# MaxMax2016/MixGAN-TTS

Hardware: AMD Instinct MI355X
Metric: denoiser steps/sec (80-mel, L=1000 frames, B=16 per GPU) (higher is better)
Workload: dtype f32

## Files before the change

mixgan-tts_amd/csrc/denoiser.hip:

```cpp
#include "denoiser_common.h"
#include "resblock_fused.h"
#include "resblock_split.h"
#include "pointwise_fused.h"
#include "denoiser_persist.h"
#include "denoiser_persist16.h"
#include "denoiser_team16.h"
#include <atomic>
#include <cstdlib>
#include <cstring>

struct EpiCond {
    struct Params {
        float *out;
        const float *bias;
        const float *x;
        const float *vec;
        int C;
    };
    template <int WM, int NNB>
    static __device__ __forceinline__ void run(const Params &p, f32x16 (&acc)[WM][NNB], int b, int mrow0, int l0w,
                                               int lane, int Lout)
    {
        const int h = lane >> 5, c = lane & 31;
#pragma unroll
// ... 401 lines not shown
    a.sig_save = sig_save;
    a.tnh_save = tnh_save;
    a.L = L;
    a.first = 1;
    const bool vec4 = (L % 4 == 0) && (((uintptr_t)cond & 15) == 0);
    launch_res_layer(a, B, L, nsave == 4, vec4, (hipStream_t)stream);
    MG_LAUNCH_CHECK();
    return MG_OK;
}

struct PostSample {
    const float *coef1, *coef2, *logvar;
    const float *noise;
    unsigned long long seed, noise_stream;
    float *x0_out;
    int n_steps, clip;
    const float *cproj;
    float *cproj_out;
    const float *step_vectors;
    int step_index, step_count;
};

static unsigned *g_host_err = nullptr, *g_host_err_dev = nullptr;
static std::atomic<int> g_host_err_state{0};

unsigned *mg_host_err_device_ptr()
{
    int s = g_host_err_state.load();
    if (s == 0) {
        static std::atomic_flag busy = ATOMIC_FLAG_INIT;
        if (busy.test_and_set()) return nullptr;
        void *h = nullptr, *dptr = nullptr;
        if (hipHostMalloc(&h, 64, hipHostMallocMapped | hipHostMallocPortable) == hipSuccess && h) {
            std::memset(h, 0, 64);
            if (hipHostGetDevicePointer(&dptr, h, 0) == hipSuccess && dptr) {
                g_host_err = (unsigned *)h;
                g_host_err_dev = (unsigned *)dptr;
                g_host_err_state.store(1);
            } else {
                (void)hipHostFree(h);
            }
        }
        (void)hipGetLastError();
        busy.clear();
        s = g_host_err_state.load();
    }
    return s == 1 ? g_host_err_dev : nullptr;
}

extern "C" unsigned mg_persist_error(int clear)
{
    if (g_host_err_state.load() != 1) {
        (void)mg_host_err_device_ptr();
        if (g_host_err_state.load() != 1) return 0u;
    }
    const unsigned v = __atomic_load_n(g_host_err, __ATOMIC_ACQUIRE);
    if (clear && v) __atomic_store_n(g_host_err, 0u, __ATOMIC_RELEASE);
    return v;
}

int mg_device_cus()
{
    static std::atomic<int> cus[64];
    int dev = 0;
    if (hipGetDevice(&dev) != hipSuccess || dev < 0 || dev >= 64) return 256;
    int n = cus[dev].load();
    if (n == 0) {
        if (hipDeviceGetAttribute(&n, hipDeviceAttributeMultiprocessorCount, dev) != hipSuccess || n <= 0) n = 256;
        cus[dev].store(n);
    }
    return n;
}

unsigned mg_persist_spin_limit()
{
    if (const char *e = std::getenv("MG_PERSIST_SPIN_LIMIT")) {
        const long v = std::atol(e);
        if (v > 0) return (unsigned)v;
    }
    return DP_SPIN_LIMIT;
}
static unsigned long long *g_persist_dbg = nullptr;
extern "C" void mg_debug_persist_stamps(unsigned long long *device_buffer) { g_persist_dbg = device_buffer; }

struct StepVecAt {
    size_t emb, h1pre, h1, s, dvec, hvec, total;
};
static inline StepVecAt den_stepvec_layout(const mg_denoiser_dims *d, size_t rows)
{
    const size_t C = d->channels, NL = d->n_layers;
    StepVecAt w;
    size_t p = 0;
    auto take = [&](size_t n) {
        size_t at = p;
        p += mg_align_up(n, 64);
        return at;
    };
    w.emb = take(rows * C);
    w.h1pre = take(rows * 4 * C);
    w.h1 = take(rows * 4 * C);
    w.s = take(rows * C);
    w.dvec = take(NL * rows * C);
    w.hvec = d->multi_speaker ? take(NL * rows * C) : w.dvec;
    w.total = p;
    return w;
}

template <class At>
static int den_step_vectors(const mg_denoiser_dims *d, const DenLayout &o, const float *packed, const int64_t *t,
                            const float *spk, float *ws, const At &w, int B, hipStream_t st, int spk_rows = 0)
{
    const int C = d->channels, H = d->cond_channels, NL = d->n_layers;
    const float *lay0 = packed + o.layers;
    hipLaunchKernelGGL(step_embed_kernel, dim3(mg_cdiv(B * (C / 2), 256)), dim3(256), 0, st, t, packed + o.freq,
                       ws + w.emb, B, C);
    MG_LAUNCH_CHECK();
    MG_TRY(small_linear(packed + o.mlp0, 0, ws + w.emb, ws + w.h1, 0, nullptr, 0, ws + w.h1pre, B, 4 * C, C, 1, 1, st));
    MG_TRY(small_linear(packed + o.mlp2, 0, ws + w.h1, ws + w.s, 0, nullptr, 0, nullptr, B, C, 4 * C, 1, 0, st));
    MG_TRY(small_linear(lay0 + o.l_wd, (long)o.layer_stride, ws + w.s, ws + w.dvec, (long)B * C, nullptr, 0, nullptr, B,
                        C, C, NL, 0, st));
    if (d->multi_speaker)
        MG_TRY(small_linear(lay0 + o.l_wp, (long)o.layer_stride, spk, ws + w.hvec, (long)B * C, ws + w.dvec,
                            (long)B * C, nullptr, B, C, H, NL, 0, st, spk_rows));
    return MG_OK;
}

extern "C" size_t mg_denoiser_step_vectors_floats(const mg_denoiser_dims *d, int n, int B)
{
    if (den_check(d) != MG_OK || n <= 0 || B <= 0) return 0;
    return den_stepvec_layout(d, (size_t)n * B).total;
}

extern "C" int mg_denoiser_step_vectors(const mg_denoiser_dims *d, const float *packed, const int64_t *t, const float *spk,
                                        float *vectors, size_t vectors_floats, int n, int B, void *stream)
{
    MG_TRY(den_check(d));
    if (!packed || !t || !vectors) return MG_ERR_ARG;
    if (d->multi_speaker && !spk) return MG_ERR_ARG;
    if (n <= 0 || B <= 0) return MG_ERR_SHAPE;
    const StepVecAt w = den_stepvec_layout(d, (size_t)n * B);
    if (vectors_floats < w.total) return MG_ERR_WORKSPACE;
    const DenLayout o = den_layout(d, 0);
    return den_step_vectors(d, o, packed, t, spk, vectors, w, n * B, (hipStream_t)stream, B);
}

static int denoiser_forward(const mg_denoiser_dims *d, const float *packed, const float *x_t, const int64_t *t,
                            const float *cond, const float *spk, float *out, float *ws, size_t ws_floats, int B,
                            int L, int mode, const PostSample *post, void *stream);

extern "C" int mg_denoiser_fwd(const mg_denoiser_dims *d, const float *packed, const float *x_t, const int64_t *t,
                               const float *cond, const float *spk, float *out, float *ws, size_t ws_floats, int B,
                               int L, int mode, void *stream)
{
    return denoiser_forward(d, packed, x_t, t, cond, spk, out, ws, ws_floats, B, L, mode, nullptr, stream);
}

extern "C" int mg_denoiser_psample(const mg_denoiser_dims *d, const float *packed, const float *x_t, const int64_t *t,
                                   const float *cond, const float *spk, const float *coef1, const float *coef2,
                                   const float *logvar, int n_steps, const float *noise, unsigned long long seed,
                                   unsigned long long noise_stream, int clip, float *x_prev, float *x0_out,
                                   const mg_sampling_loop *loop, float *ws, size_t ws_floats, int B, int L, int mode,
                                   void *stream)
{
    const float *cproj = loop ? loop->cproj : nullptr;
    float *cproj_out = loop ? loop->cproj_out : nullptr;
    const float *step_vectors = loop ? loop->step_vectors : nullptr;
// ... 83 lines not shown
struct DenFwdPins {
    int nt;
    int solo;
    int team;
};
static DenFwdPins den_fwd_pins()
{
    const char *ne = std::getenv("MG_PERSIST_NT"), *se = std::getenv("MG_PERSIST_SOLO");
    const char *te = std::getenv("MG_PERSIST_TEAM");
    return DenFwdPins{ne ? std::atoi(ne) : 0, !(se && se[0] == '0'), te ? std::atoi(te) : -1};
}

static DenFwdPlan den_fwd_plan(const mg_denoiser_dims *d, int B, int L, int mode, int cproj_mode, bool loop_vectors,
                               int cus)
{
    const bool save = mode & MG_FWD_SAVE, split = mode & MG_FWD_SPLIT, has_p16 = mode & MG_FWD_P16;
    const int C = d->channels, H = d->cond_channels, M = d->mel_bins, NL = d->n_layers;
    const DenFwdPins pin = den_fwd_pins();
    static const bool force_generic = std::getenv("MG_DENOISER_GENERIC") != nullptr;
    DenFwdPlan p{};
    p.fused = !force_generic && C == RB_C && H == RB_C;
    int nt = (long)mg_cdiv(L, 64) * B > 128 ? 64 : 32;
    if (nt == 32 && has_p16 && !save && (long)mg_cdiv(L, 32) * B <= 128) nt = 16;
    bool wide32 = nt == 32 && save && (long)mg_cdiv(L, 32) * B <= 256;
    bool eight64 = false;
    if (pin.nt == 32 || pin.nt == 64 || pin.nt == 328 || (pin.nt == 16 && has_p16 && !save)) {
        nt = pin.nt == 328 ? 32 : pin.nt;
        wide32 = pin.nt == 328;
    }
    if (pin.nt == 864) {
        nt = 64;
        eight64 = true;
    }
    if (nt == 16 && mg_cdiv(L, 16) > 128) nt = 32;
    if (nt != 32) wide32 = false;
    const bool solo32 = pin.solo && nt == 32 && !wide32 && !save && (long)mg_cdiv(L, 32) * B <= cus &&
                        mg_cdiv(L, 32) <= cus / 4;
    int team = 0;
    if (nt == 16 && !save && den_ws(d, B, L, save).team != 0 && pin.team != 0) {
        const long tiles16 = (long)mg_cdiv(L, 16) * B;
        if (tiles16 * 4 <= cus && pin.team != 2) team = 4;
        else if (tiles16 * 2 <= cus && pin.team != 4) team = 2;
    }
    const bool solo16 = pin.solo && nt == 16 && team == 0 && (long)mg_cdiv(L, 16) * B <= cus && mg_cdiv(L, 16) <= cus / 4;
    p.tiles_per_b = mg_cdiv(L, nt);
    const int chain_cap = (nt == 64 || wide32 || solo32 || solo16) ? cus / 4 : cus / 2;
    const bool persist = p.fused && !split && M <= 96 && den_persist_allowed(NL, p.tiles_per_b, chain_cap);
    p.own_vectors = !(persist && loop_vectors);
    if (!persist) return p;
    mg_fwd_plan &k = p.k;
    k.path = MG_PLAN_SINGLE;
    k.nt = nt;
    k.team = team;
    if (team) {
        k.family = MG_PLAN_TEAM16;
        k.waves = 16 / team;
        k.solo = team == 4;
    } else if (nt == 16) {
        k.family = MG_PLAN_PERSIST16;
        k.waves = 4;
        k.solo = solo16;
    } else {
        k.family = MG_PLAN_PERSIST;
        k.waves = eight64 || wide32 ? 8 : 4;
        k.solo = (nt == 64 && !eight64) || solo32;
    }
    k.cproj_mode = save ? 0 : cproj_mode;
    k.grid = p.tiles_per_b * B * (team ? team : 1);
    k.block = k.waves * 64;
    return p;
}

extern "C" int mg_denoiser_fwd_plan(const mg_denoiser_dims *d, int B, int L, int mode, int cproj_mode, int cus,
                                    mg_fwd_plan *out)
{
    MG_TRY(den_check(d));
    if (!out || cproj_mode < 0 || cproj_mode > 2 || ((mode & MG_FWD_SPLIT) && (mode & MG_FWD_SAVE))) return MG_ERR_ARG;
    if (B <= 0 || L <= 0) return MG_ERR_SHAPE;
    *out = den_fwd_plan(d, B, L, mode, cproj_mode, false, cus > 0 ? cus : mg_device_cus()).k;
    return MG_OK;
}

typedef void (*DenFwdKernel)(PersistArgs);
template <int NT, bool V, bool T, bool S, int NWV, int CPM = 0, bool SOLO = false>
constexpr DenFwdKernel dpk = denoiser_persist_kernel<NT, V, T, S, NWV, CPM, SOLO>;
struct DpForm {
    DenFwdKernel save[2];
    DenFwdKernel cpm[3][2];
    DenFwdKernel timing[3];
};
static const DpForm dp_forms[5] = {
    {{dpk<64, false, false, true, 4>, dpk<64, true, false, true, 4>},
     {{dpk<64, false, false, false, 4, 0>, dpk<64, true, false, false, 4, 0>},
      {dpk<64, false, false, false, 4, 1>, dpk<64, true, false, false, 4, 1>},
      {dpk<64, false, false, false, 4, 2>, dpk<64, true, false, false, 4, 2>}},
     {dpk<64, true, true, false, 4, 0>, nullptr, dpk<64, true, true, false, 4, 2>}},
    {{dpk<64, false, false, true, 8>, dpk<64, true, false, true, 8>},
     {{dpk<64, false, false, false, 8, 0>, dpk<64, true, false, false, 8, 0>},
      {dpk<64, false, false, false, 8, 1>, dpk<64, true, false, false, 8, 1>},
      {dpk<64, false, false, false, 8, 2>, dpk<64, true, false, false, 8, 2>}},
     {dpk<64, true, true, false, 8, 0>, nullptr, nullptr}},
    {{dpk<32, false, false, true, 8>, dpk<32, true, false, true, 8>},
     {{dpk<32, false, false, false, 8, 0>, dpk<32, true, false, false, 8, 0>},
      {dpk<32, false, false, false, 8, 1>, dpk<32, true, false, false, 8, 1>},
      {dpk<32, false, false, false, 8, 2>, dpk<32, true, false, false, 8, 2>}},
     {nullptr, nullptr, nullptr}},
    {{nullptr, nullptr},
     {{dpk<32, false, false, false, 4, 0, true>, dpk<32, true, false, false, 4, 0, true>},
      {dpk<32, false, false, false, 4, 1, true>, dpk<32, true, false, false, 4, 1, true>},
      {dpk<32, false, false, false, 4, 2, true>, dpk<32, true, false, false, 4, 2, true>}},
     {nullptr, nullptr, nullptr}},
    {{dpk<32, false, false, true, 4>, dpk<32, true, false, true, 4>},
     {{dpk<32, false, false, false, 4, 0>, dpk<32, true, false, false, 4, 0>},
      {dpk<32, false, false, false, 4, 1>, dpk<32, true, false, false, 4, 1>},
      {dpk<32, false, false, false, 4, 2>, dpk<32, true, false, false, 4, 2>}},
     {dpk<32, true, true, false, 4, 0>, nullptr, nullptr}},
};
static const DenFwdKernel dp16_kernels[2][2] = {
    {denoiser_persist16_kernel<false, false>, denoiser_persist16_kernel<true, false>},
    {denoiser_persist16_kernel<false, true>, denoiser_persist16_kernel<true, true>}};
static const DenFwdKernel team16_kernels[2][2] = {
    {denoiser_team16_kernel<false, 2>, denoiser_team16_kernel<true, 2>},
    {denoiser_team16_kernel<false, 4>, denoiser_team16_kernel<true, 4>}};

static DenFwdKernel den_fwd_kernel(const mg_fwd_plan &k, bool save, bool stamps, bool vec4)
{
    if (k.family == MG_PLAN_TEAM16) return team16_kernels[k.team == 4][vec4];
    if (k.family == MG_PLAN_PERSIST16) return dp16_kernels[k.solo != 0][vec4];
    const DpForm &f = dp_forms[k.nt == 64 ? (k.waves == 8) : k.waves == 8 ? 2 : k.solo ? 3 : 4];
    if (save) return f.save[vec4];
    if (stamps && vec4 && f.timing[k.cproj_mode]) return f.timing[k.cproj_mode];
    return f.cpm[k.cproj_mode][vec4];
}

struct DpPair {
    int b_split;
    const float *x_t, *cond;
    float *out, *ws;
    const DenWs *w;
};

static PersistArgs den_persist_args(const mg_denoiser_dims *d, const float *packed, const DenLayout &o,
                                    const DenFwdPlan &p, const float *x_t, const int64_t *t, const float *cond,
                                    float *out, float *ws, const DenWs &w, int B, int L, bool save,
                                    const PostSample *post, const DpPair *pair)
{
    const int C = d->channels, NL = d->n_layers;
    const bool p16 = p.k.nt == 16;
    float *const sws = pair ? pair->ws : save ? ws : nullptr;
    const DenWs &sw = pair ? *pair->w : w;
    PersistArgs a;
    a.x_t = x_t;
    a.cond = cond;
    a.cproj = post ? post->cproj : nullptr;
    a.cproj_out = post ? post->cproj_out : nullptr;
    a.in_w = packed + (p16 ? o.in_w16 : o.in_w);
    a.in_b = packed + o.in_b;
    a.layers = packed + o.layers;
    a.layer_stride = o.layer_stride;
    a.l_wc = o.l_wc;
    a.l_w3 = o.l_w3;
    a.l_wo = o.l_wo;
    a.l_bc = o.l_bc;
    a.l_b3 = o.l_b3;
    a.l_bo = o.l_bo;
    a.p16layers = pair ? nullptr : packed + o.p16layers;
    a.p16layer_stride = pair ? 0 : o.p16layer_stride;
    a.p_wc = pair ? 0 : o.p_wc;
    a.p_w3 = pair ? 0 : o.p_w3;
    a.p_wo = pair ? 0 : o.p_wo;
    a.skip_w = packed + (p16 ? o.skip_w16 : o.skip_w);
    a.skip_b = packed + o.skip_b;
    a.out_w = packed + (p16 ? o.out_w16 : o.out_w);
    a.out_b = packed + o.out_b;
    a.hvec = ws + w.hvec;
    a.dvec = ws + w.dvec;
    a.vec_rows = 0;
    if (!p.own_vectors) {
        const StepVecAt v = den_stepvec_layout(d, (size_t)post->step_count * B);
        a.hvec = post->step_vectors + v.hvec + (size_t)post->step_index * B * C;
        a.dvec = post->step_vectors + v.dvec + (size_t)post->step_index * B * C;
        a.vec_rows = post->step_count * B;
    }
    a.out = out;
    a.t = t;
    a.coef1 = post ? post->coef1 : nullptr;
    a.coef2 = post ? post->coef2 : nullptr;
    a.logvar = post ? post->logvar : nullptr;
    a.noise = post ? post->noise : nullptr;
    a.seed = post ? post->seed : 0ull;
    a.noise_stream = post ? post->noise_stream : 0ull;
    a.x0_out = post ? post->x0_out : nullptr;
    a.gran = reinterpret_cast<dp_u64 *>(ws + w.gran);
    a.team = p.k.team ? reinterpret_cast<dp_u64 *>(ws + w.team) : nullptr;
    a.sync = reinterpret_cast<unsigned *>(ws + w.sync);
    a.host_err = mg_host_err_device_ptr();
    a.spin_limit = mg_persist_spin_limit();
    a.B = B;
    a.L = L;
    a.M = d->mel_bins;
    a.NL = NL;
    a.tiles_per_b = p.tiles_per_b;
    a.post = post ? 1 : 0;
    a.clip = post ? post->clip : 0;
    a.n_steps = post ? post->n_steps : 1;
    a.rsNL = 1.0f / sqrtf((float)NL);
    a.dbg = pair ? nullptr : g_persist_dbg;
    const char *we = a.dbg ? std::getenv("MG_PERSIST_DBG_WAVE") : nullptr;
    a.dbg_wave = we ? std::atoi(we) & 7 : 0;
    if (a.dbg_wave >= p.k.waves) a.dbg_wave = 0;
    a.x0_save = sws ? sws + sw.x0 : nullptr;
    a.y_save = sws ? sws + sw.y : nullptr;
// ... 87 lines not shown
            a.dvec = ws + w.dvec + (size_t)l * B * C;
            a.h_save = save ? ws + w.h + (size_t)l * w.act_stride : nullptr;
            a.g_save = save ? ws + w.g + (size_t)l * w.act_stride : nullptr;
            a.sig_save = save ? ws + w.sig + (size_t)l * w.act_stride : nullptr;
            a.tnh_save = save ? ws + w.tnh + (size_t)l * w.act_stride : nullptr;
            a.L = L;
            a.first = (l == 0);
            prof_mark(st, 0);
            launch_res_layer(a, B, L, save != 0, vec4, st);
            prof_mark(st, 1);
            MG_LAUNCH_CHECK();
            float *tmp = (l == 0) ? xc : xa;
            xa = xb;
            xb = tmp;
        }
    } else {
        if (w.x0 != w.x) MG_TRY(copy_d2d(ws + w.x, ws + w.x0, (size_t)B * C * L, st));
        for (int l = 0; l < NL; ++l) {
            const float *lp = lay0 + (size_t)l * o.layer_stride;
            float *hbuf = ws + w.h + (size_t)l * w.act_stride;
            float *gbuf = ws + w.g + (size_t)l * w.act_stride;
            {
                ConvShape s{B, H, L, L, 1, 1, 0, C, 0, 0};
                EpiCond::Params ep{hbuf, lp + o.l_bc, ws + w.x, ws + w.hvec + (size_t)l * B * C, C};
                MG_TRY(conv_launch<EpiCond>(s, cond, nullptr, lp + o.l_wc, ep, st));
            }
            {
                ConvShape s{B, C, L, L, 3, 1, 1, 2 * C, 0, 0};
                EpiGate::Params ep{gbuf, lp + o.l_b3, save ? ws + w.sig + (size_t)l * w.act_stride : nullptr,
                                   save ? ws + w.tnh + (size_t)l * w.act_stride : nullptr, C};
                prof_mark(st, 0);
                MG_TRY(conv_launch<EpiGate>(s, hbuf, nullptr, lp + o.l_w3, ep, st));
                prof_mark(st, 1);
            }
            {
                ConvShape s{B, C, L, L, 1, 1, 0, 2 * C, 0, 0};
                EpiResSkip::Params ep{ws + w.x, ws + w.skip, lp + o.l_bo, ws + w.dvec + (size_t)l * B * C, C, l == 0};
                MG_TRY(conv_launch<EpiResSkip>(s, gbuf, nullptr, lp + o.l_wo, ep, st));
            }
        }
    }
    if (fused && M <= 128) {
        TailArgs ta{ws + w.skip, packed + o.skip_w, packed + o.skip_b, packed + o.out_w, packed + o.out_b,
                    save ? ws + w.y : nullptr, out, 1.0f / sqrtf((float)NL), M, L, mg_cdiv(L, RB_NT)};
        hipLaunchKernelGGL(denoiser_tail_kernel, dim3((unsigned)(ta.tiles_per_b * B)), dim3(512), 0, st, ta);
        MG_LAUNCH_CHECK();
        return post ? psample_tail(*post, out, x_t, t, final_out, reinterpret_cast<unsigned *>(ws + w.sync), B, M, L, st) : MG_OK;
    }
    {
        ConvShape s{B, C, L, L, 1, 1, 0, C, 0, 0};
        EpiBiasAct::Params ep{ws + w.y, packed + o.skip_b, nullptr, 1.0f / sqrtf((float)NL), C, MG_ACT_RELU, 0, 0, nullptr, 0.f};
        MG_TRY(conv_launch<EpiBiasAct>(s, ws + w.skip, nullptr, packed + o.skip_w, ep, st));
    }
    {
        ConvShape s{B, C, L, L, 1, 1, 0, M, 0, 0};
        EpiBiasAct::Params ep{out, packed + o.out_b, nullptr, 1.f, M, MG_ACT_NONE, 0, 0, nullptr, 0.f};
        MG_TRY(conv_launch<EpiBiasAct>(s, ws + w.y, nullptr, packed + o.out_w, ep, st));
    }
    return post ? psample_tail(*post, out, x_t, t, final_out, reinterpret_cast<unsigned *>(ws + w.sync), B, M, L, st) : MG_OK;
}

static int denoiser_forward(const mg_denoiser_dims *d, const float *packed, const float *x_t, const int64_t *t,
                            const float *cond, const float *spk, float *out, float *ws, size_t ws_floats, int B,
                            int L, int mode, const PostSample *post, void *stream)
{
    const int save = mode & MG_FWD_SAVE;
    const int split = mode & MG_FWD_SPLIT;
    if (split && save) return MG_ERR_ARG;
    MG_TRY(den_check(d));
    if (!packed || !x_t || !t || !cond || !out || !ws) return MG_ERR_ARG;
    if (d->multi_speaker && !spk) return MG_ERR_ARG;
    if (B <= 0 || L <= 0) return MG_ERR_SHAPE;
    const DenWs w = den_ws(d, B, L, save);
    if (ws_floats < w.total) return MG_ERR_WORKSPACE;
    hipStream_t st = (hipStream_t)stream;
    const DenLayout o = den_layout(d, (split ? MG_DEN_SPLIT : 0) | (mode & MG_FWD_P16 ? MG_DEN_P16 : 0));
    const int cproj_mode = post && post->cproj ? 2 : post && post->cproj_out ? 1 : 0;
    const DenFwdPlan p = den_fwd_plan(d, B, L, mode, cproj_mode, post && post->step_vectors, mg_device_cus());
    if (p.own_vectors) MG_TRY(den_step_vectors(d, o, packed, t, spk, ws, w, B, st));
    if (p.k.path == MG_PLAN_PER_LAYER)
        return den_fwd_layers(d, packed, o, x_t, t, cond, out, ws, w, B, L, save, split, p.fused, post, stream);
    const PersistArgs a = den_persist_args(d, packed, o, p, x_t, t, cond, out, ws, w, B, L, save, post, nullptr);
    const bool vec4 = (L % 4 == 0) && (((uintptr_t)cond & 15) == 0) && (((uintptr_t)a.cproj & 15) == 0);
    const DenFwdKernel kern = den_fwd_kernel(p.k, save, g_persist_dbg != nullptr, vec4);
    if (!kern) return MG_ERR_ARG;
    prof_mark(st, 0);
    hipLaunchKernelGGL(kern, dim3((unsigned)p.k.grid), dim3((unsigned)p.k.block), 0, st, a);
    prof_mark(st, 1);
    MG_LAUNCH_CHECK();
    return MG_OK;
}

extern "C" int mg_denoiser_fwd_pair(const mg_denoiser_dims *d, const float *packed, const float *x_tA, const int64_t *tA,
                                    const float *x_tB, const int64_t *tB, const float *cond, const float *spk,
                                    const float *condB, const float *spkB, float *outA, float *outB, float *wsA,
                                    size_t wsA_floats, float *wsB, size_t wsB_floats, int Bh, int L, void *stream)
{
    if (!condB) condB = cond;
    if (!spkB) spkB = spk;
    MG_TRY(den_check(d));
    if (!packed || !x_tA || !tA || !x_tB || !tB || !cond || !outA || !outB || !wsA || !wsB) return MG_ERR_ARG;
    if (d->multi_speaker && !spk) return MG_ERR_ARG;
    if (Bh <= 0 || L <= 0) return MG_ERR_SHAPE;
    const int C = d->channels, H = d->cond_channels, M = d->mel_bins, NL = d->n_layers;
    DenFwdPlan p{};
    p.tiles_per_b = mg_cdiv(L, 64);
    if (C != RB_C || H != RB_C || M > 96 || !den_persist_allowed(NL, p.tiles_per_b, mg_device_cus() / 4)) return MG_ERR_SHAPE;
    const DenWs wA = den_ws(d, 2 * Bh, L, 0), wB = den_ws(d, Bh, L, 1);
    if (wsA_floats < wA.total || wsB_floats < wB.total) return MG_ERR_WORKSPACE;
    hipStream_t st = (hipStream_t)stream;
    const DenLayout o = den_layout(d, 0);
    MG_TRY(den_step_vectors(d, o, packed, tA, spk, wsA, wA, Bh, st));
    MG_TRY(den_step_vectors(d, o, packed, tB, spkB, wsB, wB, Bh, st));
    const int waves = den_fwd_pins().nt == 864 ? 8 : 4;
    p.k = mg_fwd_plan{MG_PLAN_SINGLE, MG_PLAN_PERSIST, 64, waves, waves == 4, 0, 0, p.tiles_per_b * 2 * Bh, waves * 64};
    p.own_vectors = true;
    const DpPair pb{Bh, x_tB, condB, outB, wsB, &wB};
    const PersistArgs a = den_persist_args(d, packed, o, p, x_tA, nullptr, cond, outA, wsA, wA, 2 * Bh, L, false, nullptr, &pb);
    const bool vec4 = (L % 4 == 0) && (((uintptr_t)cond & 15) == 0) && (((uintptr_t)condB & 15) == 0);
    hipLaunchKernelGGL(den_fwd_kernel(p.k, true, false, vec4), dim3((unsigned)p.k.grid), dim3((unsigned)p.k.block), 0, st, a);
    MG_LAUNCH_CHECK();
    return MG_OK;
}
```

mixgan-tts_amd/csrc/denoiser_persist.h:

```cpp
#pragma once
#include "common.h"
#include "resblock_fused.h"

#define DP_SPIN_LIMIT (1u << 21)
#define DP_F_ROLES 1
#define DP_F_WITHHOLD 2

typedef unsigned long long dp_u64;
typedef __attribute__((address_space(1))) dp_u64 dp_gu64;
typedef __attribute__((address_space(1))) unsigned dp_gu32;

struct PersistArgs {
    const float *x_t;
    const float *cond;
    const float *cproj;
    float *cproj_out;
    const float *in_w, *in_b;
    const float *layers;
    size_t layer_stride, l_wc, l_w3, l_wo, l_bc, l_b3, l_bo;
    const float *p16layers;
    size_t p16layer_stride, p_wc, p_w3, p_wo;
    const float *skip_w, *skip_b, *out_w, *out_b;
    const float *hvec, *dvec;
    int vec_rows;
// ... 89 lines not shown
#pragma unroll
                for (int i = 0; i < NMB; ++i)
#pragma unroll
                    for (int j = 0; j < NNB; ++j)
                        acc[i][j] = __builtin_amdgcn_mfma_f32_32x32x2f32(ring[u][i][e], bb[u & 1][j][e], acc[i][j], 0, 0, 0);
                if (NMB * NNB < 4) __builtin_amdgcn_sched_barrier(0);
            }
            __builtin_amdgcn_sched_barrier(0);
        }
    }
}

template <int NTC, class F>
__device__ __forceinline__ void dp_store_block(float *T, int ch0, int col, int hh, F val)
{
#pragma unroll
    for (int q = 0; q < 4; ++q) {
        float *base = T + ((((ch0 >> 3) + q) * NTC + col) << 3);
        const f32x2 lo = {val(4 * q + 0), val(4 * q + 2)}, hi = {val(4 * q + 1), val(4 * q + 3)};
        *reinterpret_cast<f32x2 *>(base + 2 * hh) = lo;
        *reinterpret_cast<f32x2 *>(base + 4 + 2 * hh) = hi;
    }
}

__device__ __forceinline__ void dp_philox(unsigned long long seed, unsigned long long offset, unsigned long long idx,
                                          unsigned (&r)[4])
{
    unsigned c0 = (unsigned)idx, c1 = (unsigned)(idx >> 32), c2 = (unsigned)offset, c3 = (unsigned)(offset >> 32);
    unsigned k0 = (unsigned)seed, k1 = (unsigned)(seed >> 32);
#pragma unroll
    for (int i = 0; i < 10; ++i) {
        const unsigned long long p0 = (unsigned long long)0xD2511F53u * c0, p1 = (unsigned long long)0xCD9E8D57u * c2;
        const unsigned n0 = (unsigned)(p1 >> 32) ^ c1 ^ k0, n1 = (unsigned)p1, n2 = (unsigned)(p0 >> 32) ^ c3 ^ k1,
                       n3 = (unsigned)p0;
        c0 = n0; c1 = n1; c2 = n2; c3 = n3;
        k0 += 0x9E3779B9u;
        k1 += 0xBB67AE85u;
    }
    r[0] = c0; r[1] = c1; r[2] = c2; r[3] = c3;
}

__device__ __forceinline__ float dp_normal(unsigned long long seed, unsigned long long offset, unsigned long long idx)
{
    unsigned r[4];
    dp_philox(seed, offset, idx, r);
    const float u1 = ((float)r[0] + 1.0f) * 2.3283064365386963e-10f;
    const float u2 = (float)r[1] * 2.3283064365386963e-10f;
    return sqrtf(-2.0f * __logf(u1)) * __cosf(6.283185307179586f * u2);
}

#define DP_RLX_AGENT __ATOMIC_RELAXED, __HIP_MEMORY_SCOPE_AGENT

__device__ __forceinline__ void dp_fail(unsigned *sync, unsigned *host_err, unsigned code)
{
    __hip_atomic_store(sync + 1, code, DP_RLX_AGENT);
    if (host_err) __hip_atomic_store(host_err, code, __ATOMIC_RELAXED, __HIP_MEMORY_SCOPE_SYSTEM);
    __builtin_amdgcn_fence(__ATOMIC_RELEASE, "agent");
}
__device__ __forceinline__ bool dp_failed(unsigned *sync)
{
    __builtin_amdgcn_fence(__ATOMIC_ACQUIRE, "agent");
    return __hip_atomic_load(sync + 1, DP_RLX_AGENT) != 0u;
}
#define DP_STAMP(k) do { if (TIMING && tid == 64 * a.dbg_wave) a.dbg[((size_t)tile * (a.NL + 2) + stamp_row) * 12 + (k)] = clock64(); } while (0)

template <int NT, int RW>
__device__ __forceinline__ void dp_cproj_fetch(const float *cp, float *cl, int w, int lane, int l0, int L)
{
    constexpr int LPR = NT / 4;
    constexpr int RPI = 64 / LPR;
    const int rsub = lane / LPR, c4 = lane - rsub * LPR;
    unsigned off = (unsigned)(((RW * w + rsub) * L + min(l0 + 4 * c4, L - 4)) * 4);
    asm volatile("" : "+v"(off));
    float *dst = cl + (size_t)RW * w * NT;
    const unsigned at = (unsigned)(size_t)(__attribute__((address_space(3))) void *)dst;
#pragma unroll
    for (int it = 0; it < RW / RPI; ++it) {
        const float *gi = cp + (size_t)it * RPI * L;
        const unsigned m = __builtin_amdgcn_readfirstlane(at + (unsigned)(it * RPI * NT * 4));
        asm volatile("s_mov_b32 m0, %0\n\ts_nop 0\n\tglobal_load_lds_dwordx4 %1, %2" : : "s"(m), "v"(off), "s"(gi) : "memory");
    }
}

template <int NT, bool VEC4, bool TIMING = false, bool SAVE = false, int NWV = NT / 8, int CPM = 0, bool SOLO = false>
__global__ __launch_bounds__(NWV * 64, ((NT == 64 && NWV == 4) || SOLO) ? 1 : 2) void denoiser_persist_kernel(PersistArgs a)
{
    static_assert(!SOLO || (NT == 32 && NWV == 4), "SOLO is the one-per-CU build of the 4-wave 32-frame form");
    static_assert(!(CPM && SAVE), "the saving forward computes its projections and keeps none");
    constexpr bool READP = CPM == 2, WRITEP = CPM == 1;
#ifndef DP_DIST_SOLO
#define DP_DIST_SOLO 2
#endif
    constexpr int DBIG = ((NT == 64 && NWV == 4) || SOLO) ? DP_DIST_SOLO : DP_DIST_BIG;
#ifndef DP_ONEPASS_WHEN
#define DP_ONEPASS_WHEN (MB == 2 && ((NT == 64 && NWV == 4) || SOLO))
#endif
    static_assert((NT == 32 && (NWV == 4 || NWV == 8)) || (NT == 64 && (NWV == 8 || NWV == 4)),
                  "tile widths: 32 frames (4 waves, two workgroups per CU; or 8 waves, one per CU) or 64 (8 waves, one)");
    constexpr int NTHR = NWV * 64, NW = NWV;
    constexpr bool TWO_PER_CU = NT == 32 && NWV == 4;
    constexpr int MB = 8 / NW;
    constexpr bool ONEPASS = DP_ONEPASS_WHEN;
    constexpr int NNB = NT / 32;
    constexpr int NC = NT, NH = NT + 2;
    __shared__ __attribute__((aligned(16))) float lds[RB_C * (NC + NH)];
    __shared__ unsigned s_tile, s_dead, s_launch;
    float *condT = lds;
    float *hT = lds + RB_C * NC;

    const int tid = threadIdx.x, lane = tid & 63, w = tid >> 6;
    const int hh = lane >> 5, c32 = lane & 31;
    const int L = a.L;

    const int n_tiles = a.tiles_per_b * a.B;
    const unsigned hw_id = __builtin_amdgcn_s_getreg((31 << 11) | 4);
    const int role = (TWO_PER_CU && (a.flags & DP_F_ROLES)) ? (int)(hw_id & 1u) : 0;
    if (tid == 0) {
        const int nA = (TWO_PER_CU && (a.flags & DP_F_ROLES)) ? (a.B / 2) * a.tiles_per_b : n_tiles;
        const int n_mine = role == 0 ? nA : n_tiles - nA;
        unsigned tk = __hip_atomic_fetch_add(a.sync + (role ? 16 : 0), 1u, DP_RLX_AGENT);
        int tl;
        if ((int)tk < n_mine) tl = (role == 0 ? 0 : nA) + (int)tk;
        else {
            tk = __hip_atomic_fetch_add(a.sync + (role ? 0 : 16), 1u, DP_RLX_AGENT);
            tl = (role == 0 ? nA : 0) + (int)tk;
        }
        s_tile = (unsigned)tl;
        s_launch = __hip_atomic_load(a.sync + 2, DP_RLX_AGENT);
        s_dead = 0u;
    }
    __syncthreads();
    const int tile = min((int)s_tile, n_tiles - 1);
    const unsigned launch_no = s_launch;
    const int bg = tile / a.tiles_per_b, jt = tile - bg * a.tiles_per_b;
    const bool second = a.b_split > 0 && bg >= a.b_split;
    const int b = second ? bg - a.b_split : bg;
    const int Bp = a.b_split > 0 ? (second ? a.B - a.b_split : a.b_split) : a.B;
    const bool do_save = SAVE && (a.b_split == 0 || second);
    const float *const x_in = second ? a.x_t2 : a.x_t;
    float *const x_out = second ? a.out2 : a.out;
    const int l0 = jt * NT;
    const bool has_left = jt > 0, has_right = jt + 1 < a.tiles_per_b;
    int stamp_row = 0;
    DP_STAMP(0);
    if (TIMING && tid == 0) {
        a.dbg[((size_t)tile * (a.NL + 2)) * 12 + 2] = hw_id;
        a.dbg[((size_t)tile * (a.NL + 2)) * 12 + 3] = __builtin_amdgcn_s_getreg((31 << 11) | 20);
    }

    {
        const float *cb = (second ? a.cond2 : a.cond) + (size_t)b * RB_C * L;
        if (READP) {
            if (VEC4) dp_cproj_fetch<NT, 32 * MB>(a.cproj + (size_t)b * a.NL * RB_C * L, lds, w, lane, l0, L);
        } else if (VEC4) {
#pragma unroll
            for (int k = 0; k < 64 * NT / NTHR; ++k) {
                const int idx = tid + k * NTHR;
                const int row = idx / (NT / 4), c4 = idx - row * (NT / 4);
                const int f0 = l0 + 4 * c4;
                const bool ok = f0 < L;
                const f32x4 v = *reinterpret_cast<const f32x4 *>(cb + (size_t)row * L + min(f0, L - 4));
#pragma unroll
                for (int e = 0; e < 4; ++e) condT[dp_at<NC>(row, 4 * c4 + e)] = ok ? v[e] : 0.f;
            }
        } else {
#pragma unroll
            for (int k = 0; k < 256 * NT / NTHR; ++k) {
                const int idx = tid + k * NTHR;
                const int row = idx / NT, cc = idx - row * NT;
                const int f = l0 + cc;
                const float v = cb[(size_t)row * L + min(f, L - 1)];
                condT[dp_at<NC>(row, cc)] = f < L ? v : 0.f;
            }
        }
        const float *xb = x_in + (size_t)b * a.M * L;
#pragma unroll
        for (int k = 0; k < 96 * NT / NTHR; ++k) {
            const int idx = tid + k * NTHR;
            const int row = idx / NT, c = idx - row * NT;
            const int f = l0 + c;
            const float v = xb[(size_t)min(row, a.M - 1) * L + min(f, L - 1)];
            hT[dp_at<NH>(row, c)] = (row < a.M && f < L) ? v : 0.f;
        }
    }

    f32x16 st[2 * MB][NNB];
    const int rbase = 32 * MB * w;
    auto row_of = [&](int i, int r) { return rbase + 32 * i + 8 * (r >> 2) + 4 * hh + (r & 3); };
#pragma unroll
    for (int i = 0; i < MB; ++i)
#pragma unroll
        for (int j = 0; j < NNB; ++j)
#pragma unroll
            for (int r = 0; r < 16; ++r) {
                st[i][j][r] = a.in_b[row_of(i, r)];
                st[MB + i][j][r] = 0.f;
            }
    __syncthreads();
    {
        f32x16 acc[MB][NNB];
        const f32x4 *ap[MB];
#pragma unroll
        for (int i = 0; i < MB; ++i) {
            ap[i] = reinterpret_cast<const f32x4 *>(a.in_w) + (size_t)(MB * w + i) * 12 * 64 + lane;
#pragma unroll
            for (int j = 0; j < NNB; ++j) acc[i][j] = st[i][j];
        }
        dp_mfma_loop<MB, NNB, NH, DpIterHead>(acc, ap, hT + c32 * 8 + hh * 4);
#pragma unroll
        for (int i = 0; i < MB; ++i)
#pragma unroll
            for (int j = 0; j < NNB; ++j)
#pragma unroll
                for (int r = 0; r < 16; ++r) st[i][j][r] = fmaxf(acc[i][j][r], 0.f);
    }
    (void)0;
    DP_STAMP(1);
    bool fvalid[NNB];
    const size_t bbase = (size_t)b * RB_C * L;
    auto save_block = [&](float *dst, int ch0, int j, auto val) {
        const int f = l0 + 32 * j + c32;
        if (f < L) {
#pragma unroll
            for (int r = 0; r < 16; ++r) dst[bbase + (size_t)(ch0 + 8 * (r >> 2) + 4 * hh + (r & 3)) * L + f] = val(r);
        }
    };
#pragma unroll
    for (int j = 0; j < NNB; ++j) fvalid[j] = l0 + 32 * j + c32 < L;
    if (SAVE && do_save) {
#pragma unroll
        for (int i = 0; i < MB; ++i)
#pragma unroll
            for (int j = 0; j < NNB; ++j) save_block(a.x0_save, rbase + 32 * i, j, [&](int r) { return st[i][j][r]; });
    }
    dp_gu64 *const gran = (dp_gu64 *)a.gran;

    for (int l = 0; l < a.NL; ++l) {
        const float *lp = a.layers + (size_t)l * a.layer_stride;
        const size_t vrows = a.vec_rows ? (size_t)a.vec_rows : (size_t)Bp;
        const float *hv = (second ? a.hvec2 : a.hvec) + ((size_t)l * vrows + b) * RB_C;
        const float *dv = (second ? a.dvec2 : a.dvec) + ((size_t)l * vrows + b) * RB_C;
        const unsigned epoch = launch_no * ((unsigned)a.NL + 1u) + (unsigned)l + 1u;
        const int par = l & 1;
        stamp_row = l + 1;
        DP_STAMP(0);

        f32x16 acc1[MB][NNB];
        if (READP && VEC4) {
            asm volatile("s_waitcnt vmcnt(0)" ::: "memory");
#pragma unroll
            for (int i = 0; i < MB; ++i)
#pragma unroll
                for (int j = 0; j < NNB; ++j)
#pragma unroll
                    for (int r = 0; r < 16; ++r) acc1[i][j][r] = lds[row_of(i, r) * NT + 32 * j + c32];
        } else if (READP) {
            const float *cp = a.cproj + ((size_t)b * a.NL + l) * RB_C * L;
#pragma unroll
            for (int i = 0; i < MB; ++i)
#pragma unroll
                for (int j = 0; j < NNB; ++j) {
                    unsigned lo = (unsigned)((rbase + 4 * hh) * L + min(l0 + 32 * j + c32, L - 1));
                    asm volatile("" : "+v"(lo));
#pragma unroll
                    for (int r = 0; r < 16; ++r) acc1[i][j][r] = cp[lo + (unsigned)((32 * i + 8 * (r >> 2) + (r & 3)) * L)];
                }
        } else {
#pragma unroll
            for (int i = 0; i < MB; ++i)
#pragma unroll
                for (int j = 0; j < NNB; ++j)
#pragma unroll
                    for (int r = 0; r < 16; ++r) acc1[i][j][r] = lp[a.l_bc + row_of(i, r)];
            const f32x4 *wc = reinterpret_cast<const f32x4 *>(lp + a.l_wc);
            const f32x4 *ap[MB];
#pragma unroll
            for (int i = 0; i < MB; ++i) ap[i] = wc + (size_t)(MB * w + i) * 32 * 64 + lane;
            dp_mfma_loop<MB, NNB, NC, DpIterK1, (MB * NNB >= 4 ? DBIG : 3)>(acc1, ap, condT + c32 * 8 + hh * 4);
            if (WRITEP) {
                float *co = a.cproj_out + ((size_t)b * a.NL + l) * RB_C * L;
                unsigned lo = (unsigned)((rbase + 4 * hh) * L + l0 + c32);
                asm volatile("" : "+v"(lo));
#pragma unroll
                for (int i = 0; i < MB; ++i)
#pragma unroll
                    for (int j = 0; j < NNB; ++j)
                        if (l0 + 32 * j + c32 < L) {
#pragma unroll
                            for (int r = 0; r < 16; ++r)
                                co[lo + (unsigned)((32 * i + 8 * (r >> 2) + (r & 3)) * L + 32 * j)] = acc1[i][j][r];
                        }
            }
        }
#pragma unroll
        for (int i = 0; i < MB; ++i)
#pragma unroll
            for (int j = 0; j < NNB; ++j)
#pragma unroll
                for (int r = 0; r < 16; ++r) acc1[i][j][r] += st[i][j][r] + hv[row_of(i, r)];
        DP_STAMP(1);
        f32x16 acc2[MB][2][NNB];
#pragma unroll
        for (int p = 0; p < MB; ++p)
#pragma unroll
            for (int r = 0; r < 16; ++r) {
                const int ch = row_of(p, r);
                const float bg = lp[a.l_b3 + ch], bf = lp[a.l_b3 + RB_C + ch];
#pragma unroll
                for (int j = 0; j < NNB; ++j) {
                    acc2[p][0][j][r] = bg;
                    acc2[p][1][j][r] = bf;
                }
            }
        __syncthreads();
        DP_STAMP(2);
#pragma unroll
        for (int i = 0; i < MB; ++i)
#pragma unroll
            for (int j = 0; j < NNB; ++j)
            {
                dp_store_block<NH>(hT, rbase + 32 * i, 1 + 32 * j + c32, hh,
                                   [&](int r) { return fvalid[j] ? acc1[i][j][r] : 0.f; });
                if (SAVE && do_save) save_block(a.h_save + (size_t)l * a.act_stride, rbase + 32 * i, j, [&](int r) { return acc1[i][j][r]; });
            }
        if (READP && VEC4 && l + 1 < a.NL)
            dp_cproj_fetch<NT, 32 * MB>(a.cproj + ((size_t)b * a.NL + l + 1) * RB_C * L, lds, w, lane, l0, L);
        __syncthreads();
        DP_STAMP(3);

        if (w < 2) {
            bool go = w == 0 ? has_left : has_right;
            if ((a.flags & DP_F_WITHHOLD) && w == 0 && jt == 1) go = false;
            if (go) {
                const int dst_tile = w == 0 ? tile - 1 : tile + 1;
                const int col = w == 0 ? 1 : NT;
                dp_gu64 *g = gran + (((size_t)par * n_tiles + dst_tile) * 2 + (w == 0 ? 1 : 0)) * RB_C;
#pragma unroll
                for (int k = 0; k < 4; ++k) {
                    const int row = lane + 64 * k;
                    const dp_u64 v = ((dp_u64)epoch << 32) | (dp_u64)__float_as_uint(hT[dp_at<NH>(row, col)]);
                    __hip_atomic_store(g + row, v, DP_RLX_AGENT);
                }
            }
        }

        const f32x4 *w3 = reinterpret_cast<const f32x4 *>(lp + a.l_w3);
        const f32x4 *ap2[MB][2];
#pragma unroll
        for (int p = 0; p < MB; ++p) {
            ap2[p][0] = w3 + (size_t)(2 * (MB * w + p)) * 96 * 64 + lane;
            ap2[p][1] = w3 + (size_t)(2 * (MB * w + p) + 1) * 96 * 64 + lane;
        }
        if (ONEPASS) {
            dp_mfma_loop<2 * MB, NNB, NH, DpIterCentre, DBIG>(reinterpret_cast<f32x16 (&)[2 * MB][NNB]>(acc2),
                                                              reinterpret_cast<const f32x4 *const (&)[2 * MB]>(ap2),
                                                              hT + c32 * 8 + hh * 4);
        } else {
#pragma unroll
            for (int p = 0; p < MB; ++p)
                dp_mfma_loop<2, NNB, NH, DpIterCentre, (2 * NNB >= 4 ? DBIG : 3)>(acc2[p], ap2[p], hT + c32 * 8 + hh * 4);
        }
        DP_STAMP(4);

        if (w < 2) {
            const bool from = w == 0 ? has_left : has_right;
            const int col = w == 0 ? 0 : NT + 1;
            unsigned v[4] = {0u, 0u, 0u, 0u};
            if (from && s_dead == 0u) {
                dp_gu64 *g = gran + (((size_t)par * n_tiles + tile) * 2 + w) * RB_C;
                unsigned spins = 0;
                for (;;) {
                    bool ok = true;
#pragma unroll
                    for (int k = 0; k < 4; ++k) {
                        const dp_u64 x = __hip_atomic_load(g + lane + 64 * k, DP_RLX_AGENT);
                        v[k] = (unsigned)x;
                        ok &= (unsigned)(x >> 32) == epoch;
                    }
                    if (__all(ok)) break;
                    if (++spins > a.spin_limit) {
                        if (lane == 0) {
                            dp_fail(a.sync, a.host_err, 1u + (unsigned)l);
                            s_dead = 1u;
                        }
                        break;
                    }
                    __builtin_amdgcn_s_sleep(8);
                }
            }
#pragma unroll
            for (int k = 0; k < 4; ++k) hT[dp_at<NH>(lane + 64 * k, col)] = from ? __uint_as_float(v[k]) : 0.f;
        }
        DP_STAMP(5);
        __syncthreads();
        DP_STAMP(6);

        if (ONEPASS) {
            dp_mfma_loop<2 * MB, NNB, NH, DpIterOuter, DBIG>(reinterpret_cast<f32x16 (&)[2 * MB][NNB]>(acc2),
                                                             reinterpret_cast<const f32x4 *const (&)[2 * MB]>(ap2),
                                                             hT + c32 * 8 + hh * 4);
        } else {
#pragma unroll
            for (int p = 0; p < MB; ++p)
                dp_mfma_loop<2, NNB, NH, DpIterOuter, (2 * NNB >= 4 ? DBIG : 3)>(acc2[p], ap2[p], hT + c32 * 8 + hh * 4);
        }
        DP_STAMP(7);
        __syncthreads();
        DP_STAMP(8);
#pragma unroll
        for (int p = 0; p < MB; ++p)
#pragma unroll
            for (int j = 0; j < NNB; ++j)
            {
                if (SAVE && do_save) {
#pragma unroll
                    for (int r = 0; r < 16; ++r) {
                        acc2[p][0][j][r] = mg_sigmoid(acc2[p][0][j][r]);
                        acc2[p][1][j][r] = mg_tanh(acc2[p][1][j][r]);
                    }
                    const size_t lo = (size_t)l * a.act_stride;
                    save_block(a.sig_save + lo, rbase + 32 * p, j, [&](int r) { return acc2[p][0][j][r]; });
                    save_block(a.tnh_save + lo, rbase + 32 * p, j, [&](int r) { return acc2[p][1][j][r]; });
                    save_block(a.g_save + lo, rbase + 32 * p, j, [&](int r) { return acc2[p][0][j][r] * acc2[p][1][j][r]; });
                    dp_store_block<NH>(hT, rbase + 32 * p, 32 * j + c32, hh, [&](int r) { return acc2[p][0][j][r] * acc2[p][1][j][r]; });
                } else {
                    dp_store_block<NH>(hT, rbase + 32 * p, 32 * j + c32, hh,
                                       [&](int r) { return mg_sigmoid(acc2[p][0][j][r]) * mg_tanh(acc2[p][1][j][r]); });
                }
            }
#pragma unroll
        for (int i = 0; i < MB; ++i)
#pragma unroll
            for (int j = 0; j < NNB; ++j)
#pragma unroll
                for (int r = 0; r < 16; ++r) {
                    const int row = row_of(i, r);
                    st[i][j][r] += lp[a.l_bo + row] + dv[row];
                    st[MB + i][j][r] += lp[a.l_bo + RB_C + row];
                }
        DP_STAMP(9);
        __syncthreads();
        DP_STAMP(10);

        {
            const f32x4 *wo = reinterpret_cast<const f32x4 *>(lp + a.l_wo);
            const f32x4 *ap[2 * MB];
#pragma unroll
            for (int i = 0; i < MB; ++i) {
                ap[i] = wo + (size_t)(MB * w + i) * 32 * 64 + lane;
                ap[MB + i] = wo + (size_t)(8 + MB * w + i) * 32 * 64 + lane;
            }
            dp_mfma_loop<2 * MB, NNB, NH, DpIterK1, (2 * MB * NNB >= 4 ? DBIG : 3)>(st, ap, hT + c32 * 8 + hh * 4);
        }
        DP_STAMP(11);
#pragma unroll
        for (int i = 0; i < MB; ++i)
#pragma unroll
            for (int j = 0; j < NNB; ++j)
#pragma unroll
                for (int r = 0; r < 16; ++r) st[i][j][r] *= 0.70710678118654752440f;
    }

    stamp_row = a.NL + 1;
    DP_STAMP(0);
    __syncthreads();
#pragma unroll
    for (int i = 0; i < MB; ++i)
#pragma unroll
        for (int j = 0; j < NNB; ++j)
            {
                dp_store_block<NH>(hT, rbase + 32 * i, 32 * j + c32, hh, [&](int r) { return st[MB + i][j][r] * a.rsNL; });
                if (SAVE && do_save) save_block(a.skip_save, rbase + 32 * i, j, [&](int r) { return st[MB + i][j][r]; });
            }
    __syncthreads();
    {
        f32x16 acc[MB][NNB];
        const f32x4 *ap[MB];
#pragma unroll
        for (int i = 0; i < MB; ++i) {
            ap[i] = reinterpret_cast<const f32x4 *>(a.skip_w) + (size_t)(MB * w + i) * 32 * 64 + lane;
#pragma unroll
            for (int j = 0; j < NNB; ++j)
#pragma unroll
                for (int r = 0; r < 16; ++r) acc[i][j][r] = a.skip_b[row_of(i, r)];
        }
        dp_mfma_loop<MB, NNB, NH, DpIterK1>(acc, ap, hT + c32 * 8 + hh * 4);
#pragma unroll
        for (int i = 0; i < MB; ++i)
#pragma unroll
            for (int j = 0; j < NNB; ++j)
            {
                dp_store_block<NC>(condT, rbase + 32 * i, 32 * j + c32, hh, [&](int r) { return fmaxf(acc[i][j][r], 0.f); });
                if (SAVE && do_save) save_block(a.y_save, rbase + 32 * i, j, [&](int r) { return fmaxf(acc[i][j][r], 0.f); });
            }
    }
    __syncthreads();
    const int mblocks = (a.M + 31) / 32;
    for (int task = w; task < mblocks * NNB; task += NW) {
        const int mb = task / NNB, nb = task - mb * NNB;
        f32x16 o[1][1];
#pragma unroll
        for (int r = 0; r < 16; ++r) {
            const int row = 32 * mb + 8 * (r >> 2) + 4 * hh + (r & 3);
            o[0][0][r] = row < a.M ? a.out_b[row] : 0.f;
        }
        const f32x4 *const ap[1] = {reinterpret_cast<const f32x4 *>(a.out_w) + (size_t)mb * 32 * 64 + lane};
        dp_mfma_loop<1, 1, NC, DpIterK1>(o, ap, condT + (32 * nb + c32) * 8 + hh * 4);
        const int f = l0 + 32 * nb + c32;
        const size_t bo = (size_t)b * a.M * L;
        const bool bad = dp_failed(a.sync);
        const float poison = __builtin_nanf("");
        if (!a.post) {
#pragma unroll
            for (int r = 0; r < 16; ++r) {
                const int row = 32 * mb + 8 * (r >> 2) + 4 * hh + (r & 3);
                if (row < a.M && f < L) x_out[bo + (size_t)row * L + f] = bad ? poison : o[0][0][r];
            }
        } else {
            long tb = (long)a.t[b];
            tb = tb < 0 ? 0 : (tb >= a.n_steps ? a.n_steps - 1 : tb);
            const float c1 = a.coef1[tb], c2 = a.coef2[tb];
            const float sg = tb == 0 ? 0.f : __expf(0.5f * a.logvar[tb]);
// ... 35 lines not shown
```

Before: 373.2.

## Prefetch per-layer bias and step vectors into LDS via async global_load_lds

Adds a per-wave LDS staging area. The next layer's hvec, dvec, b3 and bo vectors are loaded into it asynchronously with global_load_lds_dwordx4, issued at the end of the current layer. The layer loop then reads these values as vectorized f32x4 LDS loads instead of scattered scalar global loads inside the accumulator updates. This applies only to the 64-frame 4-wave form and the SOLO form. A plain fallback is kept for misaligned pointers, and a debug query reports which path ran. The cost is extra LDS per block, an added vmcnt wait each layer, and inline asm that sets m0 by hand.

```diff
diff --git a/mixgan-tts_amd/csrc/denoiser.hip b/mixgan-tts_amd/csrc/denoiser.hip
--- a/mixgan-tts_amd/csrc/denoiser.hip
+++ b/mixgan-tts_amd/csrc/denoiser.hip
@@ -507,6 +507,8 @@
 }
 static unsigned long long *g_persist_dbg = nullptr;
 extern "C" void mg_debug_persist_stamps(unsigned long long *device_buffer) { g_persist_dbg = device_buffer; }
+static std::atomic<int> g_persist_lvec{-1};
+extern "C" int mg_debug_persist_lvec() { return g_persist_lvec.load(); }
 
 struct StepVecAt {
     size_t emb, h1pre, h1, s, dvec, hvec, total;
@@ -756,13 +758,29 @@
 }
 
 typedef void (*DenFwdKernel)(PersistArgs);
-template <int NT, bool V, bool T, bool S, int NWV, int CPM = 0, bool SOLO = false>
-constexpr DenFwdKernel dpk = denoiser_persist_kernel<NT, V, T, S, NWV, CPM, SOLO>;
+template <int NT, bool V, bool T, bool S, int NWV, int CPM = 0, bool SOLO = false, bool LV = true>
+constexpr DenFwdKernel dpk = denoiser_persist_kernel<NT, V, T, S, NWV, CPM, SOLO, LV>;
 struct DpForm {
     DenFwdKernel save[2];
     DenFwdKernel cpm[3][2];
     DenFwdKernel timing[3];
 };
+struct DpPlainVec {
+    DenFwdKernel save[2];
+    DenFwdKernel cpm[3][2];
+};
+#if DP_LVEC
+static const DpPlainVec dp_plain_vec[2] = {
+    {{dpk<64, false, false, true, 4, 0, false, false>, dpk<64, true, false, true, 4, 0, false, false>},
+     {{dpk<64, false, false, false, 4, 0, false, false>, dpk<64, true, false, false, 4, 0, false, false>},
+      {dpk<64, false, false, false, 4, 1, false, false>, dpk<64, true, false, false, 4, 1, false, false>},
+      {dpk<64, false, false, false, 4, 2, false, false>, dpk<64, true, false, false, 4, 2, false, false>}}},
+    {{nullptr, nullptr},
+     {{dpk<32, false, false, false, 4, 0, true, false>, dpk<32, true, false, false, 4, 0, true, false>},
+      {dpk<32, false, false, false, 4, 1, true, false>, dpk<32, true, false, false, 4, 1, true, false>},
+      {dpk<32, false, false, false, 4, 2, true, false>, dpk<32, true, false, false, 4, 2, true, false>}}},
+};
+#endif
 static const DpForm dp_forms[5] = {
     {{dpk<64, false, false, true, 4>, dpk<64, true, false, true, 4>},
      {{dpk<64, false, false, false, 4, 0>, dpk<64, true, false, false, 4, 0>},
@@ -797,11 +815,28 @@
     {denoiser_team16_kernel<false, 2>, denoiser_team16_kernel<true, 2>},
     {denoiser_team16_kernel<false, 4>, denoiser_team16_kernel<true, 4>}};
 
-static DenFwdKernel den_fwd_kernel(const mg_fwd_plan &k, bool save, bool stamps, bool vec4)
-{
+static bool den_lvec_aligned(const PersistArgs &a)
+{
+    auto ok = [](const void *p) { return ((uintptr_t)p & 15) == 0; };
+    return ok(a.layers + a.l_b3) && ok(a.layers + a.l_bo) && a.layer_stride % 4 == 0 && ok(a.hvec) && ok(a.dvec) &&
+           ok(a.hvec2) && ok(a.dvec2);
+}
+
+static DenFwdKernel den_fwd_kernel(const mg_fwd_plan &k, bool save, bool stamps, bool vec4, bool lvec_ok)
+{
+    g_persist_lvec.store(-1);
     if (k.family == MG_PLAN_TEAM16) return team16_kernels[k.team == 4][vec4];
     if (k.family == MG_PLAN_PERSIST16) return dp16_kernels[k.solo != 0][vec4];
     const DpForm &f = dp_forms[k.nt == 64 ? (k.waves == 8) : k.waves == 8 ? 2 : k.solo ? 3 : 4];
+    if (k.waves == 4 && k.solo) {
+        g_persist_lvec.store(DP_LVEC && lvec_ok);
+#if DP_LVEC
+        if (!lvec_ok) {
+            const DpPlainVec &pv = dp_plain_vec[k.nt == 32];
+            return save ? pv.save[vec4] : pv.cpm[k.cproj_mode][vec4];
+        }
+#endif
+    }
     if (save) return f.save[vec4];
     if (stamps && vec4 && f.timing[k.cproj_mode]) return f.timing[k.cproj_mode];
     return f.cpm[k.cproj_mode][vec4];
@@ -1055,7 +1090,7 @@
         return den_fwd_layers(d, packed, o, x_t, t, cond, out, ws, w, B, L, save, split, p.fused, post, stream);
     const PersistArgs a = den_persist_args(d, packed, o, p, x_t, t, cond, out, ws, w, B, L, save, post, nullptr);
     const bool vec4 = (L % 4 == 0) && (((uintptr_t)cond & 15) == 0) && (((uintptr_t)a.cproj & 15) == 0);
-    const DenFwdKernel kern = den_fwd_kernel(p.k, save, g_persist_dbg != nullptr, vec4);
+    const DenFwdKernel kern = den_fwd_kernel(p.k, save, g_persist_dbg != nullptr, vec4, den_lvec_aligned(a));
     if (!kern) return MG_ERR_ARG;
     prof_mark(st, 0);
     hipLaunchKernelGGL(kern, dim3((unsigned)p.k.grid), dim3((unsigned)p.k.block), 0, st, a);
@@ -1091,7 +1126,7 @@
     const DpPair pb{Bh, x_tB, condB, outB, wsB, &wB};
     const PersistArgs a = den_persist_args(d, packed, o, p, x_tA, nullptr, cond, outA, wsA, wA, 2 * Bh, L, false, nullptr, &pb);
     const bool vec4 = (L % 4 == 0) && (((uintptr_t)cond & 15) == 0) && (((uintptr_t)condB & 15) == 0);
-    hipLaunchKernelGGL(den_fwd_kernel(p.k, true, false, vec4), dim3((unsigned)p.k.grid), dim3((unsigned)p.k.block), 0, st, a);
+    hipLaunchKernelGGL(den_fwd_kernel(p.k, true, false, vec4, den_lvec_aligned(a)), dim3((unsigned)p.k.grid), dim3((unsigned)p.k.block), 0, st, a);
     MG_LAUNCH_CHECK();
     return MG_OK;
 }
diff --git a/mixgan-tts_amd/csrc/denoiser_persist.h b/mixgan-tts_amd/csrc/denoiser_persist.h
--- a/mixgan-tts_amd/csrc/denoiser_persist.h
+++ b/mixgan-tts_amd/csrc/denoiser_persist.h
@@ -195,12 +195,34 @@
     }
 }
 
-template <int NT, bool VEC4, bool TIMING = false, bool SAVE = false, int NWV = NT / 8, int CPM = 0, bool SOLO = false>
+#ifndef DP_LVEC
+#define DP_LVEC 1
+#endif
+#define DP_LV_FLOATS 512
+#define DP_LV_HV 0
+#define DP_LV_DV 64
+#define DP_LV_B3 128
+#define DP_LV_BO 256
+__device__ __forceinline__ void dp_lvec_fetch(const float *hv, const float *dv, const float *b3, const float *bo, float *rec,
+                                              int w, int lane)
+{
+    asm volatile("" : "+v"(lane));
+    const int run = lane >> 4, o = 64 * w + 4 * (lane & 15);
+    const float *p0 = (run == 0 ? hv : run == 1 ? dv : run == 2 ? b3 : b3 + RB_C) + o;
+    const float *p1 = ((run & 1) ? bo + RB_C : bo) + o;
+    const unsigned at = (unsigned)(size_t)(__attribute__((address_space(3))) void *)rec;
+    const unsigned m0a = __builtin_amdgcn_readfirstlane(at), m0b = __builtin_amdgcn_readfirstlane(at + 1024u);
+    asm volatile("s_waitcnt lgkmcnt(0)\n\ts_mov_b32 m0, %0\n\ts_nop 0\n\tglobal_load_lds_dwordx4 %1, off" : : "s"(m0a), "v"(p0) : "memory");
+    asm volatile("s_mov_b32 m0, %0\n\ts_nop 0\n\tglobal_load_lds_dwordx4 %1, off" : : "s"(m0b), "v"(p1) : "memory");
+}
+
+template <int NT, bool VEC4, bool TIMING = false, bool SAVE = false, int NWV = NT / 8, int CPM = 0, bool SOLO = false, bool LV = true>
 __global__ __launch_bounds__(NWV * 64, ((NT == 64 && NWV == 4) || SOLO) ? 1 : 2) void denoiser_persist_kernel(PersistArgs a)
 {
     static_assert(!SOLO || (NT == 32 && NWV == 4), "SOLO is the one-per-CU build of the 4-wave 32-frame form");
     static_assert(!(CPM && SAVE), "the saving forward computes its projections and keeps none");
     constexpr bool READP = CPM == 2, WRITEP = CPM == 1;
+    constexpr bool LVEC = DP_LVEC && LV && ((NT == 64 && NWV == 4) || SOLO);
 #ifndef DP_DIST_SOLO
 #define DP_DIST_SOLO 2
 #endif
@@ -216,7 +238,7 @@
     constexpr bool ONEPASS = DP_ONEPASS_WHEN;
     constexpr int NNB = NT / 32;
     constexpr int NC = NT, NH = NT + 2;
-    __shared__ __attribute__((aligned(16))) float lds[RB_C * (NC + NH)];
+    __shared__ __attribute__((aligned(16))) float lds[RB_C * (NC + NH) + (LVEC ? NWV * DP_LV_FLOATS : 0)];
     __shared__ unsigned s_tile, s_dead, s_launch;
     float *condT = lds;
     float *hT = lds + RB_C * NC;
@@ -224,6 +246,8 @@
     const int tid = threadIdx.x, lane = tid & 63, w = tid >> 6;
     const int hh = lane >> 5, c32 = lane & 31;
     const int L = a.L;
+    float *const lrec = lds + RB_C * (NC + NH) + DP_LV_FLOATS * w;
+    auto lv4 = [&](int at, int i, int q) { return *reinterpret_cast<const f32x4 *>(lrec + at + 32 * i + 8 * q + 4 * hh); };
 
     const int n_tiles = a.tiles_per_b * a.B;
     const unsigned hw_id = __builtin_amdgcn_s_getreg((31 << 11) | 4);
@@ -309,6 +333,14 @@
                 st[i][j][r] = a.in_b[row_of(i, r)];
                 st[MB + i][j][r] = 0.f;
             }
+    const size_t vrows = a.vec_rows ? (size_t)a.vec_rows : (size_t)Bp;
+    auto lvec_fetch = [&](int l) {
+        const float *lp = a.layers + (size_t)l * a.layer_stride;
+        const int bu = __builtin_amdgcn_readfirstlane(b), su = __builtin_amdgcn_readfirstlane((int)second);
+        const size_t vo = ((size_t)l * vrows + bu) * RB_C;
+        dp_lvec_fetch((su ? a.hvec2 : a.hvec) + vo, (su ? a.dvec2 : a.dvec) + vo, lp + a.l_b3, lp + a.l_bo, lrec, w, lane);
+    };
+    if (LVEC) lvec_fetch(0);
     __syncthreads();
     {
         f32x16 acc[MB][NNB];
@@ -350,7 +382,6 @@
 
     for (int l = 0; l < a.NL; ++l) {
         const float *lp = a.layers + (size_t)l * a.layer_stride;
-        const size_t vrows = a.vec_rows ? (size_t)a.vec_rows : (size_t)Bp;
         const float *hv = (second ? a.hvec2 : a.hvec) + ((size_t)l * vrows + b) * RB_C;
         const float *dv = (second ? a.dvec2 : a.dvec) + ((size_t)l * vrows + b) * RB_C;
         const unsigned epoch = launch_no * ((unsigned)a.NL + 1u) + (unsigned)l + 1u;
@@ -359,6 +390,7 @@
         DP_STAMP(0);
 
         f32x16 acc1[MB][NNB];
+        if (LVEC && !(READP && VEC4)) asm volatile("s_waitcnt vmcnt(0)" ::: "memory");
         if (READP && VEC4) {
             asm volatile("s_waitcnt vmcnt(0)" ::: "memory");
 #pragma unroll
@@ -405,26 +437,41 @@
                         }
             }
         }
-#pragma unroll
-        for (int i = 0; i < MB; ++i)
-#pragma unroll
-            for (int j = 0; j < NNB; ++j)
-#pragma unroll
-                for (int r = 0; r < 16; ++r) acc1[i][j][r] += st[i][j][r] + hv[row_of(i, r)];
+        if (LVEC) {
+#pragma unroll
+            for (int i = 0; i < MB; ++i)
+#pragma unroll
+                for (int q = 0; q < 4; ++q) {
+                    const f32x4 v = lv4(DP_LV_HV, i, q);
+#pragma unroll
+                    for (int j = 0; j < NNB; ++j)
+#pragma unroll
+                        for (int e = 0; e < 4; ++e) acc1[i][j][4 * q + e] += st[i][j][4 * q + e] + v[e];
+                }
+        } else {
+#pragma unroll
+            for (int i = 0; i < MB; ++i)
+#pragma unroll
+                for (int j = 0; j < NNB; ++j)
+#pragma unroll
+                    for (int r = 0; r < 16; ++r) acc1[i][j][r] += st[i][j][r] + hv[row_of(i, r)];
+        }
         DP_STAMP(1);
         f32x16 acc2[MB][2][NNB];
-#pragma unroll
-        for (int p = 0; p < MB; ++p)
-#pragma unroll
-            for (int r = 0; r < 16; ++r) {
-                const int ch = row_of(p, r);
-                const float bg = lp[a.l_b3 + ch], bf = lp[a.l_b3 + RB_C + ch];
-#pragma unroll
-                for (int j = 0; j < NNB; ++j) {
-                    acc2[p][0][j][r] = bg;
-                    acc2[p][1][j][r] = bf;
-                }
-            }
+        if (!LVEC) {
+#pragma unroll
+            for (int p = 0; p < MB; ++p)
+#pragma unroll
+                for (int r = 0; r < 16; ++r) {
+                    const int ch = row_of(p, r);
+                    const float bg = lp[a.l_b3 + ch], bf = lp[a.l_b3 + RB_C + ch];
+#pragma unroll
+                    for (int j = 0; j < NNB; ++j) {
+                        acc2[p][0][j][r] = bg;
+                        acc2[p][1][j][r] = bf;
+                    }
+                }
+        }
         __syncthreads();
         DP_STAMP(2);
 #pragma unroll
@@ -438,6 +485,21 @@
             }
         if (READP && VEC4 && l + 1 < a.NL)
             dp_cproj_fetch<NT, 32 * MB>(a.cproj + ((size_t)b * a.NL + l + 1) * RB_C * L, lds, w, lane, l0, L);
+        if (LVEC) {
+#pragma unroll
+            for (int p = 0; p < MB; ++p)
+#pragma unroll
+                for (int q = 0; q < 4; ++q) {
+                    const f32x4 bg = lv4(DP_LV_B3, p, q), bf = lv4(DP_LV_B3 + 64, p, q);
+#pragma unroll
+                    for (int j = 0; j < NNB; ++j)
+#pragma unroll
+                        for (int e = 0; e < 4; ++e) {
+                            acc2[p][0][j][4 * q + e] = bg[e];
+                            acc2[p][1][j][4 * q + e] = bf[e];
+                        }
+                }
+        }
         __syncthreads();
         DP_STAMP(3);
 
@@ -541,16 +603,33 @@
                                        [&](int r) { return mg_sigmoid(acc2[p][0][j][r]) * mg_tanh(acc2[p][1][j][r]); });
                 }
             }
-#pragma unroll
-        for (int i = 0; i < MB; ++i)
-#pragma unroll
-            for (int j = 0; j < NNB; ++j)
-#pragma unroll
-                for (int r = 0; r < 16; ++r) {
-                    const int row = row_of(i, r);
-                    st[i][j][r] += lp[a.l_bo + row] + dv[row];
-                    st[MB + i][j][r] += lp[a.l_bo + RB_C + row];
-                }
+        if (LVEC) {
+#pragma unroll
+            for (int i = 0; i < MB; ++i)
+#pragma unroll
+                for (int q = 0; q < 4; ++q) {
+                    const f32x4 bx = lv4(DP_LV_BO, i, q), d4 = lv4(DP_LV_DV, i, q), bs = lv4(DP_LV_BO + 64, i, q);
+#pragma unroll
+                    for (int j = 0; j < NNB; ++j)
+#pragma unroll
+                        for (int e = 0; e < 4; ++e) {
+                            st[i][j][4 * q + e] += bx[e] + d4[e];
+                            st[MB + i][j][4 * q + e] += bs[e];
+                        }
+                }
+            if (l + 1 < a.NL) lvec_fetch(l + 1);
+        } else {
+#pragma unroll
+            for (int i = 0; i < MB; ++i)
+#pragma unroll
+                for (int j = 0; j < NNB; ++j)
+#pragma unroll
+                    for (int r = 0; r < 16; ++r) {
+                        const int row = row_of(i, r);
+                        st[i][j][r] += lp[a.l_bo + row] + dv[row];
+                        st[MB + i][j][r] += lp[a.l_bo + RB_C + row];
+                    }
+        }
         DP_STAMP(9);
         __syncthreads();
         DP_STAMP(10);
```

Measured after the change: 376.0 (median of 6 runs). No clear change (+0.8%).
